# PowerfulGhost/gguf-triton-kernel

Measured on AMD Instinct MI355X. Metric: effective fp16 TFLOPS (+ quant-weight GB/s) per GGUF type, higher is better.
Workload: dtype f16; 1 GPU; q8_0_4096x4096_m128; gguf_type=q8_0, N_out=4096, K=4096, parallelism=single, weight_copies=61, weight_bytes_rotated=1087373312, graphs_rotated=1

## Files before the change

### gguf-triton-kernel_amd/csrc/gguf_internal.hpp

```cpp
#pragma once
#include <hip/hip_runtime.h>
#include <stdint.h>

namespace gq {

struct Tuning {
    long long blas_min_tokens = 768;
    long long gemm_max_bytes = 1LL << 31;
    int gemm_i8 = 0;
    int fused_decode = 1;
    int decode_f8_itc = 1;
    int decode_q6_img = -1;
    int gemm_aq = 1;
    int gemm_rg = 0;
    long long gemm_splits = 0;
    int gemm_partial_f32 = 0;
    int skinny = -1;
    int skinny_rg = 0;
    int rgemm = -1;
    int sgemm = -1;
    int sgemm_splits = 0;
    int sgemm_streamk = -1;
    int rgemm_ilc = 0;
    int sgemm_full = -1;
    int kstream = -1;
    int cus = 0;
    int ablate = 0;
};
const Tuning &tuning();
int set_tuning(const char *key, long long value);
void reset_tuning();
int num_cus();

enum ActMode : int { ACT_AOS = 0, ACT_SOA = 1, ACT_DEQ = 2, ACT_I8 = 3, ACT_F8 = 4, ACT_F8DEQ = 5 };
enum ActForm : int { AF_F16 = 0, AF_I8 = 1 };

hipError_t launch_quant_blocks(int kind, const void *x, void *y, int64_t nblocks, hipStream_t s);

hipError_t launch_act_quant(int mode, const uint16_t *X, int64_t ldx, int64_t rows, int64_t K, void *out0,
                            void *out1, void *out2, hipStream_t s);
constexpr int kMaxDeqSegs = 8;
struct DeqSeg {
    const uint16_t *X;
    int64_t ldx, rows, K;
    uint16_t *xdeq;
    int64_t wg0;
};
hipError_t launch_act_quant_deq_grouped(const DeqSeg *segs, int n, hipStream_t s, int mode = ACT_DEQ);

hipError_t launch_gemv(int fmt, const uint8_t *A, const int8_t *xq, const float *xd, const float *xs, uint16_t *C,
                       int64_t M, int64_t N, int64_t K, int64_t ldc, hipStream_t s);

bool decode_fused_ok(int fmt, int64_t N, int64_t K, bool fp8 = false);
hipError_t launch_decode_fused(int fmt, const uint8_t *A, const uint16_t *X, int64_t ldx, uint16_t *C, int64_t M,
                               int64_t N, int64_t K, int64_t ldc, hipStream_t s, bool fp8 = false);

struct GemmPlan {
    int nb = 8;
    int rg = 2;
    int splits = 1;
    int chunks_per_split = 1;
    int act = AF_F16;
    int loaders = 0;
    int pf16 = 0;
    int aq = 0;
    size_t partial_bytes = 0;
};
struct GemmAct {
    const uint16_t *xdeq = nullptr;
    const int8_t *xq = nullptr;
    const float *xd = nullptr;
    int64_t ldd = 0;
    const uint16_t *xraw = nullptr;
    int64_t ldx = 0;
};
bool gemm_aq_ok(const GemmPlan &p);
bool gemm_supported(int fmt, int64_t K);
GemmPlan plan_gemm(int fmt, int64_t M, int64_t N, int64_t K, int act = AF_F16);
hipError_t launch_gemm(int fmt, const uint8_t *A, const GemmAct &x, uint16_t *C, float *partials,
                       const GemmPlan &plan, int64_t M, int64_t N, int64_t K, int64_t ldc, hipStream_t s);

hipError_t launch_gemm_reduce_f16(int nb, int rg, const uint16_t *P, uint16_t *C, int64_t M, int64_t N, int64_t ldc,
                                  int S, int tiles_x, int tiles_y, hipStream_t s);

struct RGemmPlan {
    bool ok = false;
    int nb = 8, tiles_m = 0, tiles_n = 0, splits = 1;
    size_t partial_bytes = 0;
};

RGemmPlan plan_rgemm(int64_t M, int64_t N, int64_t K);
bool rgemm_ilc(int fmt, const RGemmPlan &p);
unsigned int ilc_timeouts();
unsigned int kstream_timeouts();
int rgemm_per_cu(int fmt, int nb);
hipError_t launch_rgemm(int fmt, int aq, const uint8_t *A, const uint16_t *X, int64_t ldx, uint16_t *C, void *partials,
                        const RGemmPlan &p, int64_t M, int64_t N, int64_t K, int64_t ldc, hipStream_t s);
RGemmPlan plan_sgemm(int64_t M, int64_t N, int64_t K, int splits);
bool sgemm_ilc(const RGemmPlan &p);
hipError_t launch_sgemm(int fmt, const uint8_t *A, const uint16_t *X, uint16_t *C, void *partials, const RGemmPlan &p,
                        int64_t M, int64_t N, int64_t K, int64_t ldc, hipStream_t s);

struct SGroupItem {
    int fmt;
    const uint8_t *A;
    const uint16_t *X;
    uint16_t *C;
    int64_t ldc, M, K;
};
struct SGroupPlan {
    bool ok = false;
    int nb = 8, tiles_n = 1, blocks = 0;
    int tiles_m[16] = {}, splits[16] = {}, wg0[16] = {};
    bool streamk = false;
    int U = 0;
    int ustart[16] = {}, scap[16] = {};
    int cost[16] = {}, cstart[16] = {};
    size_t poff[16] = {};
    size_t foff[16] = {}, noff[16] = {};
    size_t partial_bytes = 0;
};
SGroupPlan plan_sgemm_grouped(const SGroupItem *items, int n, int64_t N, int splits);
hipError_t launch_sgemm_grouped(const SGroupItem *items, int n, int64_t N, const SGroupPlan &g, void *partials,
                                hipStream_t s);

struct DecodeItem {
    int fmt;
    const uint8_t *A;
    const uint16_t *X;
    int64_t ldx;
    uint16_t *C;
    int64_t ldc;
    int64_t M, K;
};
bool decode_grouped_ok(const DecodeItem *items, int n, int64_t N, bool fp8 = false);
hipError_t launch_decode_grouped(const DecodeItem *items, int n, int64_t N, hipStream_t s, bool fp8 = false);

constexpr int kMaxIdPairs = 64;
bool decode_id_ok(int fmt, int64_t M, int64_t pairs, int64_t K);
hipError_t launch_decode_id(int fmt, const uint8_t *A, const int32_t *ids, const uint16_t *B, uint16_t *C, int64_t E,
                            int64_t M, int64_t N, int64_t S, int64_t K, int64_t ldb, int64_t ldb_slot, int64_t ldc,
                            hipStream_t s);

bool decode_id_glu_ok(int fmt, int64_t M, int64_t pairs, int64_t K);
hipError_t launch_decode_id_glu(int fmt, const uint8_t *A_gate, const uint8_t *A_up, const int32_t *ids, const uint16_t *B,
// ... 60 lines not shown
```

### gguf-triton-kernel_amd/csrc/gq_capi.hip

```cpp
#include <climits>
#include <cstdio>
#include <dlfcn.h>
#include <mutex>
#include <cstdarg>
#include <cstdlib>
#include <string>

#include <rccl/rccl.h>

#include "../../include/gguf_mmq.h"
#include "gguf_blocks.hpp"
#include "gguf_internal.hpp"

namespace gq {
namespace {

Tuning g_tuning;
std::once_flag g_tuning_once;

bool parse_key(Tuning &t, const char *key, long long v)
{
    auto in = [&](std::initializer_list<long long> ok) {
        for (long long o : ok)
            if (v == o) return true;
        return false;
    };
    const std::string k = key;
    if (k == "GQ_BLAS_MIN_TOKENS") t.blas_min_tokens = v;
    else if (k == "GQ_GEMM_MAX_BYTES") {
        if (v <= 0) return false;
        t.gemm_max_bytes = v < (1LL << 31) ? v : (1LL << 31);
    } else if (k == "GQ_GEMM_I8") t.gemm_i8 = v != 0;
    else if (k == "GQ_NO_FUSED_DECODE") t.fused_decode = v == 0;
    else if (k == "GQ_DECODE_F8_ITC") t.decode_f8_itc = v != 0;
    else if (k == "GQ_SGEMM_STREAMK") t.sgemm_streamk = v < 0 ? -1 : (v != 0);
    else if (k == "GQ_DECODE_Q6_IMG") {
        if (!in({-1, 0, 1})) return false;
        t.decode_q6_img = (int)v;
    }
    else if (k == "GQ_GEMM_AQ") t.gemm_aq = v != 0;
    else if (k == "GQ_GEMM_RG") {
        if (!in({0, 1, 2})) return false;
        t.gemm_rg = (int)v;
    } else if (k == "GQ_GEMM_SPLITS") {
        if (v < 0) return false;
        t.gemm_splits = v;
    } else if (k == "GQ_GEMM_PARTIAL") t.gemm_partial_f32 = v != 0;
    else if (k == "GQ_SKINNY") {
        if (!in({-1, 0, 1})) return false;
        t.skinny = (int)v;
    } else if (k == "GQ_SKINNY_RG") {
        if (!in({0, 1, 2, 3, 4})) return false;
        t.skinny_rg = (int)v;
    } else if (k == "GQ_RGEMM") {
        if (!in({-1, 0, 1})) return false;
        t.rgemm = (int)v;
    } else if (k == "GQ_SGEMM") {
        if (!in({-1, 0, 1})) return false;
        t.sgemm = (int)v;
    } else if (k == "GQ_SGEMM_SPLITS") {
        if (v < 0 || v > 4096) return false;
        t.sgemm_splits = (int)v;
    } else if (k == "GQ_RGEMM_ILC") t.rgemm_ilc = v != 0;
    else if (k == "GQ_SGEMM_FULL") {
        t.sgemm_full = v < 0 ? -1 : (v != 0);
    } else if (k == "GQ_CUS") {
        if (v < 0 || v > 1024) return false;
        t.cus = (int)v;
    } else if (k == "GQ_KSTREAM") {
        if (!in({-1, 0, 1})) return false;
        t.kstream = (int)v;
    } else if (k == "GQ_ABLATE") t.ablate = (int)v;
    else return false;
    return true;
}

void tuning_from_env(Tuning &t)
{
    t = Tuning{};
    static const char *const keys[] = {"GQ_BLAS_MIN_TOKENS", "GQ_GEMM_MAX_BYTES", "GQ_GEMM_I8", "GQ_NO_FUSED_DECODE",
                                       "GQ_DECODE_Q6_IMG", "GQ_DECODE_F8_ITC", "GQ_GEMM_AQ", "GQ_GEMM_RG", "GQ_GEMM_SPLITS",
                                       "GQ_GEMM_PARTIAL", "GQ_SKINNY", "GQ_SKINNY_RG", "GQ_RGEMM", "GQ_SGEMM",
                                       "GQ_SGEMM_SPLITS", "GQ_SGEMM_STREAMK", "GQ_RGEMM_ILC", "GQ_SGEMM_FULL", "GQ_CUS",
                                       "GQ_KSTREAM", "GQ_ABLATE"};
    for (const char *k : keys) {
        const char *e = getenv(k);
        if (!e || !*e) continue;
        long long v;
        if (std::string(k) == "GQ_GEMM_PARTIAL") v = std::string(e) == "f32";
        else v = atoll(e);
        if (!parse_key(t, k, v)) fprintf(stderr, "gguf_mmq: ignoring %s=%s (out of range)\n", k, e);
    }
}

}

const Tuning &tuning()
{
    std::call_once(g_tuning_once, [] { tuning_from_env(g_tuning); });
    return g_tuning;
}

int set_tuning(const char *key, long long value)
{
    tuning();
    Tuning t = g_tuning;
    if (!key || !parse_key(t, key, value)) return -1;
    g_tuning = t;
    return 0;
}

void reset_tuning()
{
    tuning();
    Tuning t;
    tuning_from_env(t);
    g_tuning = t;
}

int num_cus()
{
    if (tuning().cus > 0) return tuning().cus;
    static int cached[64] = {0};
    int dev = 0;
    if (hipGetDevice(&dev) != hipSuccess || dev < 0 || dev >= 64) dev = 0;
    if (cached[dev] <= 0) {
        int n = 0;
        if (hipDeviceGetAttribute(&n, hipDeviceAttributeMultiprocessorCount, dev) != hipSuccess || n <= 0) n = 256;
        cached[dev] = n;
    }
    return cached[dev];
}

namespace {

struct TypeInfo {
// ... 1114 lines not shown
```

### gguf-triton-kernel_amd/csrc/mmq_rgemm.hip

```cpp
#include <algorithm>
#include <type_traits>

#include "gguf_blocks.hpp"
#include "gguf_internal.hpp"
#include "gguf_mfma.hpp"
#include "gguf_q8_1.hpp"

namespace gq {

#ifdef GQ_RGEMM_STAMPS
__device__ unsigned long long g_rstamps[65536][14];
#define GQ_RST(i) (st[i] = __builtin_amdgcn_s_memtime())
#else
#define GQ_RST(i) ((void)0)
#endif

__device__ unsigned int g_ilc_timeouts;

namespace {

#ifndef GQ_RGEMM_ABL
#define GQ_RGEMM_ABL 0
#endif
constexpr int ABL = GQ_RGEMM_ABL;

constexpr int RW = 8;
constexpr int RPRIO_WAVE = RW / 2;
constexpr int RRG = 2;
constexpr int RBM = 16 * RW * RRG;
constexpr int LDS_CAP = 160 * 1024;
constexpr int kSpol = 16;

template <int F> struct HImg;
template <> struct HImg<Q8_0> { static constexpr int NPH = 9; };
template <> struct HImg<Q4_K> { static constexpr int NPH = 5; };
template <> struct HImg<Q5_K> { static constexpr int NPH = 7; };
template <> struct HImg<Q3_K> { static constexpr int NPH = 5; };
template <> struct HImg<Q2_K> { static constexpr int NPH = 5; };
template <> struct HImg<Q4_0> { static constexpr int NPH = 5; };
#ifndef GQ_Q6_NPH
#define GQ_Q6_NPH 8
#endif
template <> struct HImg<Q6_K> { static constexpr int NPH = GQ_Q6_NPH; };
template <int F> __device__ __forceinline__ int hpos_swz(int r)
{
    return F == Q6_K && HImg<F>::NPH == 8 ? (r & 7) : 0;
}
template <int F> __device__ __forceinline__ uint32_t hsrc(int h, int pc)
{
    if constexpr (F == Q8_0) return 128u * h + 16u * pc;
    if constexpr (F == Q4_K) return pc == 0 ? 0u : 16u + 64u * h + 16u * (pc - 1);
    if constexpr (F == Q5_K) return pc < 3 ? 16u * pc : 48u + 64u * h + 16u * (pc - 3);
    if constexpr (F == Q3_K) return pc < 2 ? 16u * pc : (pc < 4 ? 32u + 32u * h + 16u * (pc - 2) : 94u);
    if constexpr (F == Q2_K) return pc == 0 || pc == 4 ? 0u : (pc < 3 ? 16u + 32u * h + 16u * (pc - 1) : 68u);
    if constexpr (F == Q4_0) return 64u * h + 16u * pc;
    return pc < 4 ? 64u * h + 16u * pc : (pc < 6 ? 128u + 32u * h + 16u * (pc - 4) : (pc == 6 ? 192u : 194u));
}

template <int F, int NB> struct RCfg {
    static constexpr int BN = 16 * NB;
    static constexpr int NPH = HImg<F>::NPH, HRB = 16 * NPH, SB = Layout<F>::BYTES * (256 / Layout<F>::QK);
    static constexpr int WW = 2 * 32 * HRB, WWI = WW / 1024, H0I = (32 * NPH + 63) / 64;
    static constexpr int X_OFF = RW * WW;
    static constexpr int X_BYTES = BN * 512;
    static constexpr int X_INSTR = X_BYTES / 1024;
    static constexpr int NX = X_INSTR / RW;
    static constexpr int LDS = X_OFF + X_BYTES;
    static_assert(WW % 1024 == 0 && X_INSTR % RW == 0, "whole DMA instructions per wave");
    static_assert(LDS <= LDS_CAP, "LDS budget");
};

template <int F> __device__ __forceinline__ int sub_elem(int u, int q)
{
    if constexpr (F == Q6_K) return 128 * (u >> 1) + 32 * (u & 1) + 64 * (q >> 2) + 8 * (q & 3);
    return 64 * u + 8 * q;
}

template <int F> __device__ __forceinline__ void block_piece(int kb, int j, int &u, int &q)
{
    if constexpr (F == Q6_K) {
        const int b4 = kb & 3;
        u = 2 * (kb >> 2) + (b4 & 1);
        q = 4 * (b4 >> 1) + j;
    } else {
// ... 150 lines not shown
                }
            }
#pragma unroll
            for (int g = 0; g < G; ++g) {
                if (s0 + g >= S) v[g] = (u32x4){0u, 0u, 0u, 0u};
#pragma unroll
                for (int j = 0; j < TPU; ++j) {
                    const uint32_t x0 = j == 0 ? v[g].x : v[g].z, x1 = j == 0 ? v[g].y : v[g].w;
                    acc[j][0] += h2f(x0 & 0xffffu) * up[g];
                    acc[j][1] += h2f(x0 >> 16) * up[g];
                    acc[j][2] += h2f(x1 & 0xffffu) * up[g];
                    acc[j][3] += h2f(x1 >> 16) * up[g];
                }
            }
        }
        const int64_t row = m0 + 16 * wr + 4 * (ln >> 4);
        if (row >= M) continue;
#pragma unroll
        for (int j = 0; j < TPU; ++j) {
            const int64_t tok = n0 + 16 * (TPU * u + j) + (ln & 15);
            if (tok >= N) continue;
            uint16_t *dst = C + tok * ldc + row;
            if (row + 4 <= M) {
                *(u32x2 *)dst = (u32x2){(uint32_t)f2h_bits(acc[j][0]) | ((uint32_t)f2h_bits(acc[j][1]) << 16),
                                        (uint32_t)f2h_bits(acc[j][2]) | ((uint32_t)f2h_bits(acc[j][3]) << 16)};
            } else {
                for (int e = 0; e < 4 && row + e < M; ++e) dst[e] = f2h_bits(acc[j][e]);
            }
        }
    }
}

template <int NB>
__device__ __forceinline__ void ilc_combine(uint16_t *__restrict__ C, uint16_t *__restrict__ P, int64_t M, int64_t N,
                                            int64_t ldc, const TileId &id, uint32_t nonce)
{
    constexpr int BN = 16 * NB;
    const int lane = threadIdx.x & 63, wave = __builtin_amdgcn_readfirstlane(threadIdx.x >> 6);
    const int gz = id.gz, z = id.z;
    const int64_t tile = (int64_t)id.y * id.gx + id.x;
    const IlcSync sy = ilc_sync(P, id, BN);
    asm volatile("s_waitcnt vmcnt(0)" ::: "memory");
    __syncthreads();
    if (wave == 0) {
        uint64_t *tf = sy.flags + tile * gz;
        if (lane == 0) __hip_atomic_store(tf + z, ilc_flag(nonce, gz, z), __ATOMIC_RELAXED, __HIP_MEMORY_SCOPE_AGENT);
        ilc_wait(tf, nonce, gz);
        if (lane == 0 && z == 0) __hip_atomic_store(sy.nonce + tile, nonce + 1u, __ATOMIC_RELAXED, __HIP_MEMORY_SCOPE_AGENT);
    }
    __syncthreads();
    ilc_sum<NB>(C, P, M, N, ldc, (int64_t)id.x * RBM, (int64_t)id.y * BN, tile, gz, (int64_t)id.gx * id.gy * gz, gz, z,
                gz);
}
template <int NB>
__device__ __forceinline__ void store_tile(const f32x4 (&acc)[RRG][NB], uint16_t *__restrict__ C,
                                           uint16_t *__restrict__ P, int64_t M, int64_t N, int64_t ldc, int spol,
                                           const TileId &id)
{
    constexpr int BN = 16 * NB;
    const int lane = threadIdx.x & 63, wave = __builtin_amdgcn_readfirstlane(threadIdx.x >> 6);
    const int g = lane >> 4, l16 = lane & 15;
    const int64_t m0 = (int64_t)id.x * RBM, n0 = (int64_t)id.y * BN;
    if (id.gz > 1) {
        const int64_t tile = (int64_t)id.y * id.gx + id.x;
        const int64_t bidx = tile * id.gz + id.z;
        float mx = 0.f;
#pragma unroll
        for (int rg = 0; rg < RRG; ++rg)
#pragma unroll
            for (int t = 0; t < NB; ++t)
#pragma unroll
                for (int i = 0; i < 4; ++i) mx = fmaxf(mx, fabsf(acc[rg][t][i]));
        int m = __builtin_bit_cast(int, mx);
        m = __builtin_bit_cast(int, fmaxf(__builtin_bit_cast(float, m), __builtin_bit_cast(float, __builtin_amdgcn_update_dpp(0, m, 0x111, 0xf, 0xf, true))));
        m = __builtin_bit_cast(int, fmaxf(__builtin_bit_cast(float, m), __builtin_bit_cast(float, __builtin_amdgcn_update_dpp(0, m, 0x112, 0xf, 0xf, true))));
        m = __builtin_bit_cast(int, fmaxf(__builtin_bit_cast(float, m), __builtin_bit_cast(float, __builtin_amdgcn_update_dpp(0, m, 0x114, 0xf, 0xf, true))));
        m = __builtin_bit_cast(int, fmaxf(__builtin_bit_cast(float, m), __builtin_bit_cast(float, __builtin_amdgcn_update_dpp(0, m, 0x118, 0xf, 0xf, true))));
        m = __builtin_bit_cast(int, fmaxf(__builtin_bit_cast(float, m), __builtin_bit_cast(float, __builtin_amdgcn_update_dpp(0, m, 0x142, 0xa, 0xf, true))));
        m = __builtin_bit_cast(int, fmaxf(__builtin_bit_cast(float, m), __builtin_bit_cast(float, __builtin_amdgcn_update_dpp(0, m, 0x143, 0xc, 0xf, true))));
        const uint32_t mb = (uint32_t)__builtin_amdgcn_readlane(m, 63);
        const int E = (int)((mb >> 23) & 0xff) - 127;
        const int e = E - 14 > 0 ? (E - 14 < 127 ? E - 14 : 126) : 0;
        const float down = __builtin_bit_cast(float, (uint32_t)(127 - e) << 23);
        const int64_t nblk = (int64_t)id.gx * id.gy * id.gz;
        const __amdgpu_buffer_rsrc_t prs = __builtin_amdgcn_make_buffer_rsrc(
            (void *)P, 0, (int)(uint32_t)(nblk * (RBM * BN * 2 + RW * 4)), 0x00020000);
        const uint32_t bo = (uint32_t)(bidx * (RBM * BN * 2));
        if (lane == 0) {
            const uint32_t eo = (uint32_t)(nblk * (RBM * BN * 2) + (bidx * RW + wave) * 4);
            if (spol == 2) __builtin_amdgcn_raw_buffer_store_b32((uint32_t)e, prs, eo, 0, 2);
            else if (spol == 16) __builtin_amdgcn_raw_buffer_store_b32((uint32_t)e, prs, eo, 0, 16);
            else __builtin_amdgcn_raw_buffer_store_b32((uint32_t)e, prs, eo, 0, 0);
        }
        auto pk = [down](const f32x4 &v) {
            return (u32x2){(uint32_t)f2h_bits(v[0] * down) | ((uint32_t)f2h_bits(v[1] * down) << 16),
                           (uint32_t)f2h_bits(v[2] * down) | ((uint32_t)f2h_bits(v[3] * down) << 16)};
        };
#pragma unroll
        for (int rg = 0; rg < RRG; ++rg) {
            if constexpr (NB == 1) {
                const uint32_t vo = bo + 8u * (uint32_t)((RRG * wave + rg) * 64 + lane);
                if (spol == 2) __builtin_amdgcn_raw_buffer_store_b64(pk(acc[rg][0]), prs, vo, 0, 2);
                else if (spol == 16) __builtin_amdgcn_raw_buffer_store_b64(pk(acc[rg][0]), prs, vo, 0, 16);
                else __builtin_amdgcn_raw_buffer_store_b64(pk(acc[rg][0]), prs, vo, 0, 0);
            } else {
#pragma unroll
                for (int uu = 0; uu < NB / 2; ++uu) {
                    const u32x2 lo = pk(acc[rg][2 * uu]), hi = pk(acc[rg][2 * uu + 1]);
                    const u32x4 w = {lo.x, lo.y, hi.x, hi.y};
                    const uint32_t vo = bo + 16u * (uint32_t)(((RRG * wave + rg) * (NB / 2) + uu) * 64 + lane);
                    if (spol == 2) __builtin_amdgcn_raw_buffer_store_b128(w, prs, vo, 0, 2);
                    else if (spol == 16) __builtin_amdgcn_raw_buffer_store_b128(w, prs, vo, 0, 16);
                    else __builtin_amdgcn_raw_buffer_store_b128(w, prs, vo, 0, 0);
                }
            }
        }
        return;
    }
#pragma unroll
    for (int rg = 0; rg < RRG; ++rg) {
        const int64_t row = m0 + 16 * (RRG * wave + rg) + 4 * g;
        if (row >= M) continue;
#pragma unroll
        for (int t = 0; t < NB; ++t) {
            const int64_t tok = n0 + 16 * t + l16;
            if (tok >= N) continue;
            const f32x4 v = acc[rg][t];
            uint16_t *dst = C + tok * ldc + row;
            if (row + 4 <= M) {
                *(u32x2 *)dst = (u32x2){(uint32_t)f2h_bits(v[0]) | ((uint32_t)f2h_bits(v[1]) << 16),
                                        (uint32_t)f2h_bits(v[2]) | ((uint32_t)f2h_bits(v[3]) << 16)};
            } else {
                for (int i = 0; i < 4 && row + i < M; ++i) dst[i] = f2h_bits(v[i]);
            }
        }
    }
}

template <int NB>
__device__ __forceinline__ void store_tile_rows(const f32x4 (&acc)[RRG][NB], uint16_t *__restrict__ C,
                                                const int32_t *__restrict__ rowmap, int64_t M, int64_t N, int64_t ldc,
                                                const TileId &id)
{
    const int lane = threadIdx.x & 63, wave = __builtin_amdgcn_readfirstlane(threadIdx.x >> 6);
    const int g = lane >> 4, l16 = lane & 15;
    const int64_t m0 = (int64_t)id.x * RBM;
#pragma unroll
    for (int t = 0; t < NB; ++t) {
        const int tok = 16 * t + l16;
        if (tok >= N) continue;
        uint16_t *out = C + (int64_t)rowmap[tok] * ldc;
#pragma unroll
        for (int rg = 0; rg < RRG; ++rg) {
            const int64_t row = m0 + 16 * (RRG * wave + rg) + 4 * g;
            if (row >= M) continue;
            const f32x4 v = acc[rg][t];
            uint16_t *dst = out + row;
            if (row + 4 <= M) {
                *(u32x2 *)dst = (u32x2){(uint32_t)f2h_bits(v[0]) | ((uint32_t)f2h_bits(v[1]) << 16),
                                        (uint32_t)f2h_bits(v[2]) | ((uint32_t)f2h_bits(v[3]) << 16)};
            } else {
                for (int i = 0; i < 4 && row + i < M; ++i) dst[i] = f2h_bits(v[i]);
            }
        }
    }
}

template <int F, int NB, int AQ>
__global__ __launch_bounds__(64 * RW) void rgemm_kernel(const uint8_t *__restrict__ A, const uint16_t *__restrict__ X,
                                                       int64_t ldx, uint16_t *__restrict__ C, uint16_t *__restrict__ P,
                                                       int64_t M, int64_t N, int64_t K, int64_t ldc, int spol,
                                                       int ilc_gx, int ilc_gy)
{
    using G = RCfg<F, NB>;
    __shared__ __attribute__((aligned(1024))) uint8_t lds[G::LDS];
    const int tid = threadIdx.x, lane = tid & 63;
    const int wave = __builtin_amdgcn_readfirstlane(tid >> 6);
    const bool ilc = ilc_gx > 0;
    if (wave >= RPRIO_WAVE) __builtin_amdgcn_s_setprio(1);
    const TileId tile = ilc ? ilc_tile(ilc_gx, ilc_gy) : grid_tile();
    const int64_t m0 = (int64_t)tile.x * RBM, n0 = (int64_t)tile.y * G::BN, sb = tile.z;
    const int64_t row_bytes = (K / Layout<F>::QK) * Layout<F>::BYTES;
    uint8_t *const ximg = lds + G::X_OFF;
#ifdef GQ_RGEMM_STAMPS
    unsigned long long st[14] = {};
    st[0] = __builtin_amdgcn_s_memrealtime();
    GQ_RST(1);
#endif
    const uint32_t nonce = ilc_nonce(P, tile, G::BN, ilc);

    u32x4 xv[AQ ? NB : 1];
    if constexpr (AQ != 0 && !(ABL & 2)) {
        const __amdgpu_buffer_rsrc_t xrs =
            __builtin_amdgcn_make_buffer_rsrc((void *)X, 0, (int)(uint32_t)(((N - 1) * ldx + K) * 2), 0x00020000);
#pragma unroll
        for (int ps = 0; ps < NB; ++ps) {
            const int b = 128 * ps + (tid >> 2), r = b >> 3, kb = b & 7;
            const int64_t tok = n0 + r < N ? n0 + r : N - 1;
            xv[ps] = __builtin_amdgcn_raw_buffer_load_b128(
                xrs, (uint32_t)(tok * ldx * 2) + 2u * (uint32_t)(256 * sb + 32 * kb + 8 * (lane & 3)), 0, 0);
        }
    }

    const __amdgpu_buffer_rsrc_t wrs =
        __builtin_amdgcn_make_buffer_rsrc((void *)A, 0, (int)(uint32_t)((M * row_bytes + 15) & ~(int64_t)15), 0x00020000);
    uint8_t *const wimg = lds + wave * G::WW;
    auto issue_w = [&](auto i0c, auto i1c) __attribute__((always_inline)) {
        constexpr int I0 = decltype(i0c)::value, I1 = decltype(i1c)::value;
        if constexpr (ABL & 1) return;
#pragma unroll
        for (int i = I0; i < I1; ++i) {
            const int p = 64 * i + lane, h = p / (32 * G::NPH), rem = p - h * (32 * G::NPH);
            const int r = rem / G::NPH, pc = (rem - r * G::NPH) ^ hpos_swz<F>(r);
            const int64_t row = m0 + 32 * wave + r < M ? m0 + 32 * wave + r : M - 1;
            dma16(wrs, wimg + 1024 * i, (uint32_t)(row * row_bytes) + hsrc<F>(h, pc), (uint32_t)(G::SB * sb));
        }
    };
    auto issue_x = [&]() __attribute__((always_inline)) {
        if constexpr (AQ != 0 || (ABL & 2)) return;
        const __amdgpu_buffer_rsrc_t xrs =
            __builtin_amdgcn_make_buffer_rsrc((void *)X, 0, (int)(uint32_t)(N * K * 2), 0x00020000);
#pragma unroll
        for (int i = 0; i < G::NX; ++i) {
            const int k = wave + RW * i, pp = 64 * k + lane;
            const int u = pp / (G::BN * 8), r = (pp / 8) % G::BN, qd = pp & 7, q = qd ^ act_swz(r);
            const int64_t tok = n0 + r < N ? n0 + r : N - 1;
            const uint32_t vo = (uint32_t)(tok * K * 2) + 2u * (uint32_t)sub_elem<F>(u, q);
            dma16(xrs, lds + G::X_OFF + 1024 * k, vo, (uint32_t)(512 * sb));
        }
    };
#ifndef GQ_RGEMM_WPRE
#define GQ_RGEMM_WPRE 2
#endif
    constexpr int WPRE = AQ != 0 && GQ_RGEMM_WPRE < G::WWI ? GQ_RGEMM_WPRE : G::WWI;
    issue_x();
    issue_w(std::integral_constant<int, 0>{}, std::integral_constant<int, WPRE>{});
    GQ_RST(2);

    if constexpr (AQ != 0 && !(ABL & 2)) {
#pragma unroll
        for (int ps = 0; ps < NB; ++ps) {
            const int b = 128 * ps + (tid >> 2), r = b >> 3, kb = b & 7;
            u32x4 o;
            if constexpr (AQ == 2) {
                const F8Quad fq = f8_quad(xv[ps]);
                o = (u32x4){fq.xt[0], fq.xt[1], fq.xt[2], fq.xt[3]};
            } else {
                o = deq_quad(xv[ps]);
            }
            int u, q;
            block_piece<F>(kb, lane & 3, u, q);
            *(u32x4 *)(ximg + u * (G::BN * 128) + 128 * r + 16 * (q ^ act_swz(r))) = o;
        }
    }
    issue_w(std::integral_constant<int, WPRE>{}, std::integral_constant<int, G::WWI>{});
    constexpr int WN = (ABL & 1) ? 0 : G::WWI;
    asm volatile("s_waitcnt vmcnt(%0) lgkmcnt(0)" ::"n"(WN) : "memory");
    GQ_RST(3);
    __builtin_amdgcn_s_barrier();
    GQ_RST(4);

    f32x4 acc[RRG][NB];
#pragma unroll
    for (int rg = 0; rg < RRG; ++rg)
#pragma unroll
        for (int t = 0; t < NB; ++t) acc[rg][t] = (f32x4){0.f, 0.f, 0.f, 0.f};
    constexpr int H1N = (ABL & 1) ? 0 : G::WWI - G::H0I;
    asm volatile("s_waitcnt vmcnt(%0)" ::"n"(H1N) : "memory");
    GQ_RST(5);
#pragma unroll
    for (int u = 0; u < 4 && !(ABL & 4); ++u) {
        if (u == 2) {
#ifdef GQ_RGEMM_STAMPS
            asm volatile("s_waitcnt lgkmcnt(0)" ::: "memory");
            for (int rg = 0; rg < RRG; ++rg)
                for (int t = 0; t < NB; ++t) asm volatile("" ::"v"(acc[rg][t]));
#endif
            GQ_RST(6);
            asm volatile("s_waitcnt vmcnt(0)" ::: "memory");
            GQ_RST(7);
        }
        mul_substage<F, NB>(wimg + (u >> 1) * (32 * G::HRB), ximg + u * (G::BN * 128), u, acc, 0);
    }
#ifdef GQ_RGEMM_STAMPS
    for (int rg = 0; rg < RRG; ++rg)
        for (int t = 0; t < NB; ++t) asm volatile("" ::"v"(acc[rg][t]));
#endif
    GQ_RST(8);
    if constexpr ((ABL & 4) != 0) asm volatile("s_waitcnt vmcnt(0)" ::: "memory");

    if constexpr ((ABL & 8) != 0) {
        if (acc[0][0][0] == 1234.5f) C[0] = 0;
        return;
    }
    store_tile<NB>(acc, C, P, M, N, ldc, ilc ? 16 : spol, tile);
    if (ilc && tile.gz > 1) ilc_combine<NB>(C, P, M, N, ldc, tile, nonce);
#ifdef GQ_RGEMM_STAMPS
    GQ_RST(9);
    asm volatile("s_waitcnt vmcnt(0)" ::: "memory");
    GQ_RST(10);
    st[11] = __builtin_amdgcn_s_memrealtime();
    const int wg = (int)(blockIdx.x + gridDim.x * (blockIdx.y + gridDim.y * blockIdx.z));
    st[12] = (unsigned long long)wg;
    unsigned xcc;
    asm volatile("s_getreg_b32 %0, hwreg(HW_REG_XCC_ID)" : "=s"(xcc));
    st[13] = xcc & 0xfu;
    const int id = wg * RW + wave;
    if (lane == 0 && id < 65536)
        for (int i = 0; i < 14; ++i) g_rstamps[id][i] = st[i];
#endif
}

#ifndef GQ_SGEMM_NSMAX
#define GQ_SGEMM_NSMAX 6
#endif
constexpr int SG_NSMAX = GQ_SGEMM_NSMAX;
template <int F, int NB> struct SCfg {
    static constexpr int BN = 16 * NB;
    static constexpr int NPH = HImg<F>::NPH, HRB = 16 * NPH, SB = Layout<F>::BYTES * (256 / Layout<F>::QK);
    static constexpr int W_BYTES = RBM * HRB, X_BYTES = BN * 256;
    static constexpr int SLOT = W_BYTES + X_BYTES;
    static constexpr int WH_INSTR = (RBM * NPH + 63) / 64, NWH = (WH_INSTR + RW - 1) / RW;
    static constexpr int XH_INSTR = X_BYTES / 1024, NXH = (XH_INSTR + RW - 1) / RW;
    static constexpr int NPS = ((ABL & 1) ? 0 : NWH) + ((ABL & 2) ? 0 : NXH);
    static constexpr bool PAD = WH_INSTR % RW != 0 || XH_INSTR % RW != 0 || XH_INSTR < RW;
    static constexpr int NS = (LDS_CAP - 1024) / SLOT > SG_NSMAX ? SG_NSMAX : (LDS_CAP - 1024) / SLOT;
    static constexpr int SCRATCH = NS * SLOT;
    static constexpr int LDS = SCRATCH + (PAD ? 1024 : 0);
    static_assert(NS >= 2, "two ring slots");
    static_assert(LDS <= LDS_CAP, "LDS budget");
    static_assert((NS - 2) * NPS <= 63, "vmcnt range");
};

constexpr int kMaxSParts = 16;
struct SPart {
    int fmt;
    const uint8_t *A;
    const uint16_t *X;
    uint16_t *C, *P;
    int64_t M, K, ldc;
    int tiles_m, tiles_n, splits, wg0;
    int ustart, scap;
    int cost, cstart;
    uint64_t *flags;
    uint32_t *nonce;
};
struct SParts {
    int n;
// ... 433 lines not shown
                acc[j][0] += h2f(x0 & 0xffffu) * up[k];
                acc[j][1] += h2f(x0 >> 16) * up[k];
                acc[j][2] += h2f(x1 & 0xffffu) * up[k];
                acc[j][3] += h2f(x1 >> 16) * up[k];
            }
        }
    }
    const int64_t row = m0 + 16 * wr + 4 * (lane >> 4);
    if (row >= q.M) return;
#pragma unroll
    for (int j = 0; j < TPU; ++j) {
        const int64_t tok = n0 + 16 * (TPU * u + j) + (lane & 15);
        if (tok >= a.N) continue;
        uint16_t *dst = q.C + tok * q.ldc + row;
        if (row + 4 <= q.M) {
            *(u32x2 *)dst = (u32x2){(uint32_t)f2h_bits(acc[j][0]) | ((uint32_t)f2h_bits(acc[j][1]) << 16),
                                    (uint32_t)f2h_bits(acc[j][2]) | ((uint32_t)f2h_bits(acc[j][3]) << 16)};
        } else {
            for (int e = 0; e < 4 && row + e < q.M; ++e) dst[e] = f2h_bits(acc[j][e]);
        }
    }
}

template <int F, int NB>
hipError_t launch_snb(const uint8_t *A, const uint16_t *X, uint16_t *C, void *P, const RGemmPlan &p, int64_t M,
                      int64_t N, int64_t K, int64_t ldc, hipStream_t s)
{
    static const int occ = [] {
        int n = 0;
        return hipOccupancyMaxActiveBlocksPerMultiprocessor(&n, sgemm_kernel<F, NB>, 64 * RW, 0) == hipSuccess ? n : 0;
    }();
    const int64_t blocks = (int64_t)p.tiles_m * p.tiles_n * p.splits;
    if (sgemm_ilc(p) && blocks <= (int64_t)num_cus() * occ) {
        sgemm_kernel<F, NB><<<dim3((unsigned)blocks), dim3(64 * RW), 0, s>>>(A, X, C, (uint16_t *)P, M, N, K, ldc, 16,
                                                                             tuning().sgemm_full != 0, p.tiles_m, p.tiles_n, 1);
        return hipGetLastError();
    }
#ifndef GQ_SGEMM_ZORDER
#define GQ_SGEMM_ZORDER 1
#endif
    if (GQ_SGEMM_ZORDER && p.splits > 1 && (blocks & 7) == 0 && N * K * 2 > ((int64_t)4 << 20)) {
        sgemm_kernel<F, NB><<<dim3((unsigned)blocks), dim3(64 * RW), 0, s>>>(A, X, C, (uint16_t *)P, M, N, K, ldc, kSpol,
                                                                             tuning().sgemm_full != 0, p.tiles_m, p.tiles_n, 2);
    } else {
        const dim3 grid((unsigned)p.tiles_m, (unsigned)p.tiles_n, (unsigned)p.splits);
        sgemm_kernel<F, NB><<<grid, dim3(64 * RW), 0, s>>>(A, X, C, (uint16_t *)P, M, N, K, ldc, kSpol,
                                                            tuning().sgemm_full != 0, 0, 0, 0);
    }
    hipError_t e = hipGetLastError();
    if (e != hipSuccess || p.splits == 1) return e;
    return launch_gemm_reduce_f16(NB, RRG, (const uint16_t *)P, C, M, N, ldc, p.splits, p.tiles_m, p.tiles_n, s);
}

template <int F, int NB, int AQ>
hipError_t launch_nb(const uint8_t *A, const uint16_t *X, int64_t ldx, uint16_t *C, void *P, const RGemmPlan &p,
                     int64_t M, int64_t N, int64_t K, int64_t ldc, hipStream_t s)
{
    static const int occ = [] {
        int n = 0;
        return hipOccupancyMaxActiveBlocksPerMultiprocessor(&n, rgemm_kernel<F, NB, AQ>, 64 * RW, 0) == hipSuccess ? n : 0;
    }();
    const int64_t blocks = (int64_t)p.tiles_m * p.tiles_n * p.splits;
    if (rgemm_ilc(F, p) && blocks <= (int64_t)num_cus() * occ) {
        rgemm_kernel<F, NB, AQ><<<dim3((unsigned)blocks), dim3(64 * RW), 0, s>>>(A, X, ldx, C, (uint16_t *)P, M, N, K, ldc,
                                                                                 16, p.tiles_m, p.tiles_n);
        return hipGetLastError();
    }
    const dim3 grid((unsigned)p.tiles_m, (unsigned)p.tiles_n, (unsigned)p.splits);
    rgemm_kernel<F, NB, AQ><<<grid, dim3(64 * RW), 0, s>>>(A, X, ldx, C, (uint16_t *)P, M, N, K, ldc, kSpol,
                                                           0, 0);
    hipError_t e = hipGetLastError();
    if (e != hipSuccess || p.splits == 1) return e;
    return launch_gemm_reduce_f16(NB, RRG, (const uint16_t *)P, C, M, N, ldc, p.splits, p.tiles_m, p.tiles_n, s);
}

template <int F, int AQ>
hipError_t launch_f(const uint8_t *A, const uint16_t *X, int64_t ldx, uint16_t *C, void *P, const RGemmPlan &p,
                    int64_t M, int64_t N, int64_t K, int64_t ldc, hipStream_t s)
{
    switch (p.nb) {
    case 1: return launch_nb<F, 1, AQ>(A, X, ldx, C, P, p, M, N, K, ldc, s);
    case 2: return launch_nb<F, 2, AQ>(A, X, ldx, C, P, p, M, N, K, ldc, s);
    case 4: return launch_nb<F, 4, AQ>(A, X, ldx, C, P, p, M, N, K, ldc, s);
    case 8: return launch_nb<F, 8, AQ>(A, X, ldx, C, P, p, M, N, K, ldc, s);
    default: return hipErrorInvalidValue;
    }
}

}

int rgemm_per_cu(int fmt, int nb)
{
#define GQ_RPC(F)                                                                                                      \
    switch (nb) {                                                                                                      \
    case 1: return LDS_CAP / RCfg<F, 1>::LDS;                                                                          \
    case 2: return LDS_CAP / RCfg<F, 2>::LDS;                                                                          \
    case 4: return LDS_CAP / RCfg<F, 4>::LDS;                                                                          \
    default: return LDS_CAP / RCfg<F, 8>::LDS;                                                                         \
    }
    switch (fmt) {
    case Q8_0: GQ_RPC(Q8_0)
    case Q4_K: GQ_RPC(Q4_K)
    case Q6_K: GQ_RPC(Q6_K)
    default: return 0;
    }
#undef GQ_RPC
}

RGemmPlan plan_rgemm(int64_t M, int64_t N, int64_t K)
{
    RGemmPlan p;
    if (M < 1 || N < 1 || K < 256 || K % 256 != 0) return p;
    p.nb = N > 64 ? 8 : (N > 32 ? 4 : (N > 16 ? 2 : 1));
    p.tiles_m = (int)((M + RBM - 1) / RBM);
    p.tiles_n = (int)((N + 16 * p.nb - 1) / (16 * p.nb));
    p.splits = (int)(K / 256);
    const int64_t tiles = (int64_t)p.tiles_m * p.tiles_n, nblk = tiles * p.splits;
    p.partial_bytes = p.splits > 1 ? ilc_flags_off(nblk, 16 * p.nb) + ilc_sync_bytes(nblk, tiles) : 0;
    p.ok = true;
    return p;
}

bool rgemm_ilc(int fmt, const RGemmPlan &p)
{
    if (!p.ok || p.splits < 2 || tuning().rgemm_ilc == 0) return false;
    return (int64_t)p.tiles_m * p.tiles_n * p.splits <= (int64_t)num_cus() * rgemm_per_cu(fmt, p.nb);
}

bool sgemm_ilc(const RGemmPlan &p)
{
    if (!p.ok || p.splits < 2 || tuning().rgemm_ilc == 0) return false;
    return (int64_t)p.tiles_m * p.tiles_n * p.splits <= (int64_t)num_cus();
}

unsigned int ilc_timeouts()
{
    unsigned int v = 0;
    return hipMemcpyFromSymbol(&v, HIP_SYMBOL(g_ilc_timeouts), sizeof(v)) == hipSuccess ? v : ~0u;
}

RGemmPlan plan_sgemm(int64_t M, int64_t N, int64_t K, int splits)
{
    RGemmPlan p;
    if (M < 1 || N < 1 || K < 256 || K % 256 != 0) return p;
    p.nb = N > 64 ? 8 : (N > 32 ? 4 : (N > 16 ? 2 : 1));
    p.tiles_m = (int)((M + RBM - 1) / RBM);
    p.tiles_n = (int)((N + 16 * p.nb - 1) / (16 * p.nb));
    const int64_t tiles = (int64_t)p.tiles_m * p.tiles_n, nsb = K / 256, cus = num_cus();
    int64_t S = splits > 0 ? splits : (tiles >= cus ? 1 : cus / tiles);
    if (S > nsb) S = nsb;
    p.splits = (int)(S < 1 ? 1 : S);
    const int64_t nblk = tiles * p.splits;
    p.partial_bytes = p.splits > 1 ? ilc_flags_off(nblk, 16 * p.nb) + ilc_sync_bytes(nblk, tiles) : 0;
    p.ok = true;
    return p;
}

hipError_t launch_sgemm(int fmt, const uint8_t *A, const uint16_t *X, uint16_t *C, void *partials, const RGemmPlan &p,
                        int64_t M, int64_t N, int64_t K, int64_t ldc, hipStream_t s)
{
    if (!p.ok) return hipErrorInvalidValue;
    return dispatch_fmt(fmt, [&](auto f) {
        constexpr int F = decltype(f)::value;
        switch (p.nb) {
        case 1: return launch_snb<F, 1>(A, X, C, partials, p, M, N, K, ldc, s);
        case 2: return launch_snb<F, 2>(A, X, C, partials, p, M, N, K, ldc, s);
        case 4: return launch_snb<F, 4>(A, X, C, partials, p, M, N, K, ldc, s);
        case 8: return launch_snb<F, 8>(A, X, C, partials, p, M, N, K, ldc, s);
        default: return hipErrorInvalidValue;
        }
    });
}

SortedPlan plan_sgemm_id(int64_t E, int64_t M, int64_t P, int64_t K)
{
    SortedPlan p;
    if (E < 1 || E > kMaxSortExperts || M < 1 || P < 1 || P > kMaxSortPairs || K < 256 || K % 256 != 0) return p;
    const int64_t ne = E < P ? E : P, avg = (P + ne - 1) / ne;
    p.nb = avg > 64 ? 8 : (avg > 32 ? 4 : (avg > 16 ? 2 : 1));
// ... 212 lines not shown
```

Baseline: 274.1 TFLOP/s.

## Overlap rgemm epilogue stores with the second-half MFMAs per token group

```diff
diff --git a/gguf-triton-kernel_amd/csrc/gguf_internal.hpp b/gguf-triton-kernel_amd/csrc/gguf_internal.hpp
--- a/gguf-triton-kernel_amd/csrc/gguf_internal.hpp
+++ b/gguf-triton-kernel_amd/csrc/gguf_internal.hpp
@@ -22,6 +22,7 @@
     int sgemm_splits = 0;
     int sgemm_streamk = -1;
     int rgemm_ilc = 0;
+    int rgemm_estore = -1;
     int sgemm_full = -1;
     int kstream = -1;
     int cus = 0;
@@ -91,6 +92,7 @@
 
 RGemmPlan plan_rgemm(int64_t M, int64_t N, int64_t K);
 bool rgemm_ilc(int fmt, const RGemmPlan &p);
+bool rgemm_estore(int nb);
 unsigned int ilc_timeouts();
 unsigned int kstream_timeouts();
 int rgemm_per_cu(int fmt, int nb);
diff --git a/gguf-triton-kernel_amd/csrc/gq_capi.hip b/gguf-triton-kernel_amd/csrc/gq_capi.hip
--- a/gguf-triton-kernel_amd/csrc/gq_capi.hip
+++ b/gguf-triton-kernel_amd/csrc/gq_capi.hip
@@ -62,7 +62,10 @@
         if (v < 0 || v > 4096) return false;
         t.sgemm_splits = (int)v;
     } else if (k == "GQ_RGEMM_ILC") t.rgemm_ilc = v != 0;
-    else if (k == "GQ_SGEMM_FULL") {
+    else if (k == "GQ_RGEMM_ESTORE") {
+        if (!in({-1, 0, 1})) return false;
+        t.rgemm_estore = (int)v;
+    } else if (k == "GQ_SGEMM_FULL") {
         t.sgemm_full = v < 0 ? -1 : (v != 0);
     } else if (k == "GQ_CUS") {
         if (v < 0 || v > 1024) return false;
@@ -81,7 +84,7 @@
     static const char *const keys[] = {"GQ_BLAS_MIN_TOKENS", "GQ_GEMM_MAX_BYTES", "GQ_GEMM_I8", "GQ_NO_FUSED_DECODE",
                                        "GQ_DECODE_Q6_IMG", "GQ_DECODE_F8_ITC", "GQ_GEMM_AQ", "GQ_GEMM_RG", "GQ_GEMM_SPLITS",
                                        "GQ_GEMM_PARTIAL", "GQ_SKINNY", "GQ_SKINNY_RG", "GQ_RGEMM", "GQ_SGEMM",
-                                       "GQ_SGEMM_SPLITS", "GQ_SGEMM_STREAMK", "GQ_RGEMM_ILC", "GQ_SGEMM_FULL", "GQ_CUS",
+                                       "GQ_SGEMM_SPLITS", "GQ_SGEMM_STREAMK", "GQ_RGEMM_ILC", "GQ_RGEMM_ESTORE", "GQ_SGEMM_FULL", "GQ_CUS",
                                        "GQ_KSTREAM", "GQ_ABLATE"};
     for (const char *k : keys) {
         const char *e = getenv(k);
diff --git a/gguf-triton-kernel_amd/csrc/mmq_rgemm.hip b/gguf-triton-kernel_amd/csrc/mmq_rgemm.hip
--- a/gguf-triton-kernel_amd/csrc/mmq_rgemm.hip
+++ b/gguf-triton-kernel_amd/csrc/mmq_rgemm.hip
@@ -11,8 +11,10 @@
 #ifdef GQ_RGEMM_STAMPS
 __device__ unsigned long long g_rstamps[65536][14];
 #define GQ_RST(i) (st[i] = __builtin_amdgcn_s_memtime())
+#define GQ_RST_PTR(i) (&st[i])
 #else
 #define GQ_RST(i) ((void)0)
+#define GQ_RST_PTR(i) nullptr
 #endif
 
 __device__ unsigned int g_ilc_timeouts;
@@ -30,6 +32,7 @@
 constexpr int RBM = 16 * RW * RRG;
 constexpr int LDS_CAP = 160 * 1024;
 constexpr int kSpol = 16;
+constexpr int kEstoreAutoNb = 2;
 
 template <int F> struct HImg;
 template <> struct HImg<Q8_0> { static constexpr int NPH = 9; };
@@ -286,46 +289,53 @@
     ilc_sum<NB>(C, P, M, N, ldc, (int64_t)id.x * RBM, (int64_t)id.y * BN, tile, gz, (int64_t)id.gx * id.gy * gz, gz, z,
                 gz);
 }
-template <int NB>
-__device__ __forceinline__ void store_tile(const f32x4 (&acc)[RRG][NB], uint16_t *__restrict__ C,
-                                           uint16_t *__restrict__ P, int64_t M, int64_t N, int64_t ldc, int spol,
-                                           const TileId &id)
-{
-    constexpr int BN = 16 * NB;
-    const int lane = threadIdx.x & 63, wave = __builtin_amdgcn_readfirstlane(threadIdx.x >> 6);
-    const int g = lane >> 4, l16 = lane & 15;
-    const int64_t m0 = (int64_t)id.x * RBM, n0 = (int64_t)id.y * BN;
-    if (id.gz > 1) {
-        const int64_t tile = (int64_t)id.y * id.gx + id.x;
-        const int64_t bidx = tile * id.gz + id.z;
-        float mx = 0.f;
-#pragma unroll
-        for (int rg = 0; rg < RRG; ++rg)
-#pragma unroll
-            for (int t = 0; t < NB; ++t)
-#pragma unroll
-                for (int i = 0; i < 4; ++i) mx = fmaxf(mx, fabsf(acc[rg][t][i]));
-        int m = __builtin_bit_cast(int, mx);
-        m = __builtin_bit_cast(int, fmaxf(__builtin_bit_cast(float, m), __builtin_bit_cast(float, __builtin_amdgcn_update_dpp(0, m, 0x111, 0xf, 0xf, true))));
-        m = __builtin_bit_cast(int, fmaxf(__builtin_bit_cast(float, m), __builtin_bit_cast(float, __builtin_amdgcn_update_dpp(0, m, 0x112, 0xf, 0xf, true))));
-        m = __builtin_bit_cast(int, fmaxf(__builtin_bit_cast(float, m), __builtin_bit_cast(float, __builtin_amdgcn_update_dpp(0, m, 0x114, 0xf, 0xf, true))));
-        m = __builtin_bit_cast(int, fmaxf(__builtin_bit_cast(float, m), __builtin_bit_cast(float, __builtin_amdgcn_update_dpp(0, m, 0x118, 0xf, 0xf, true))));
-        m = __builtin_bit_cast(int, fmaxf(__builtin_bit_cast(float, m), __builtin_bit_cast(float, __builtin_amdgcn_update_dpp(0, m, 0x142, 0xa, 0xf, true))));
-        m = __builtin_bit_cast(int, fmaxf(__builtin_bit_cast(float, m), __builtin_bit_cast(float, __builtin_amdgcn_update_dpp(0, m, 0x143, 0xc, 0xf, true))));
-        const uint32_t mb = (uint32_t)__builtin_amdgcn_readlane(m, 63);
-        const int E = (int)((mb >> 23) & 0xff) - 127;
-        const int e = E - 14 > 0 ? (E - 14 < 127 ? E - 14 : 126) : 0;
-        const float down = __builtin_bit_cast(float, (uint32_t)(127 - e) << 23);
+__device__ __forceinline__ int wave_exponent(float mx)
+{
+    int m = __builtin_bit_cast(int, mx);
+    m = __builtin_bit_cast(int, fmaxf(__builtin_bit_cast(float, m), __builtin_bit_cast(float, __builtin_amdgcn_update_dpp(0, m, 0x111, 0xf, 0xf, true))));
+    m = __builtin_bit_cast(int, fmaxf(__builtin_bit_cast(float, m), __builtin_bit_cast(float, __builtin_amdgcn_update_dpp(0, m, 0x112, 0xf, 0xf, true))));
+    m = __builtin_bit_cast(int, fmaxf(__builtin_bit_cast(float, m), __builtin_bit_cast(float, __builtin_amdgcn_update_dpp(0, m, 0x114, 0xf, 0xf, true))));
+    m = __builtin_bit_cast(int, fmaxf(__builtin_bit_cast(float, m), __builtin_bit_cast(float, __builtin_amdgcn_update_dpp(0, m, 0x118, 0xf, 0xf, true))));
+    m = __builtin_bit_cast(int, fmaxf(__builtin_bit_cast(float, m), __builtin_bit_cast(float, __builtin_amdgcn_update_dpp(0, m, 0x142, 0xa, 0xf, true))));
+    m = __builtin_bit_cast(int, fmaxf(__builtin_bit_cast(float, m), __builtin_bit_cast(float, __builtin_amdgcn_update_dpp(0, m, 0x143, 0xc, 0xf, true))));
+    const uint32_t mb = (uint32_t)__builtin_amdgcn_readlane(m, 63);
+    const int E = (int)((mb >> 23) & 0xff) - 127;
+    return E - 14 > 0 ? (E - 14 < 127 ? E - 14 : 126) : 0;
+}
+template <int NB> __device__ __forceinline__ float tile_absmax(const f32x4 (&acc)[RRG][NB], int t0, int t1, float mx)
+{
+#pragma unroll
+    for (int rg = 0; rg < RRG; ++rg)
+#pragma unroll
+        for (int t = t0; t < t1; ++t)
+#pragma unroll
+            for (int i = 0; i < 4; ++i) mx = fmaxf(mx, fabsf(acc[rg][t][i]));
+    return mx;
+}
+template <int NB, int SP = -1> struct PartBlock {
+    __amdgpu_buffer_rsrc_t prs;
+    uint32_t bo, eo;
+    int spol;
+    __device__ __forceinline__ PartBlock(uint16_t *P, const TileId &id, int spol_) : spol(SP < 0 ? spol_ : SP)
+    {
+        constexpr int BN = 16 * NB;
+        const int wave = __builtin_amdgcn_readfirstlane(threadIdx.x >> 6);
+        const int64_t bidx = ((int64_t)id.y * id.gx + id.x) * id.gz + id.z;
         const int64_t nblk = (int64_t)id.gx * id.gy * id.gz;
-        const __amdgpu_buffer_rsrc_t prs = __builtin_amdgcn_make_buffer_rsrc(
-            (void *)P, 0, (int)(uint32_t)(nblk * (RBM * BN * 2 + RW * 4)), 0x00020000);
-        const uint32_t bo = (uint32_t)(bidx * (RBM * BN * 2));
-        if (lane == 0) {
-            const uint32_t eo = (uint32_t)(nblk * (RBM * BN * 2) + (bidx * RW + wave) * 4);
-            if (spol == 2) __builtin_amdgcn_raw_buffer_store_b32((uint32_t)e, prs, eo, 0, 2);
-            else if (spol == 16) __builtin_amdgcn_raw_buffer_store_b32((uint32_t)e, prs, eo, 0, 16);
-            else __builtin_amdgcn_raw_buffer_store_b32((uint32_t)e, prs, eo, 0, 0);
-        }
+        prs = __builtin_amdgcn_make_buffer_rsrc((void *)P, 0, (int)(uint32_t)(nblk * (RBM * BN * 2 + RW * 4)), 0x00020000);
+        bo = (uint32_t)(bidx * (RBM * BN * 2));
+        eo = (uint32_t)(nblk * (RBM * BN * 2) + (bidx * RW + wave) * 4);
+    }
+    __device__ __forceinline__ void exponent(int e) const
+    {
+        if ((threadIdx.x & 63) != 0) return;
+        if (spol == 2) __builtin_amdgcn_raw_buffer_store_b32((uint32_t)e, prs, eo, 0, 2);
+        else if (spol == 16) __builtin_amdgcn_raw_buffer_store_b32((uint32_t)e, prs, eo, 0, 16);
+        else __builtin_amdgcn_raw_buffer_store_b32((uint32_t)e, prs, eo, 0, 0);
+    }
+    __device__ __forceinline__ void tiles(const f32x4 (&acc)[RRG][NB], int t0, int t1, float down) const
+    {
+        const int lane = threadIdx.x & 63, wave = __builtin_amdgcn_readfirstlane(threadIdx.x >> 6);
         auto pk = [down](const f32x4 &v) {
             return (u32x2){(uint32_t)f2h_bits(v[0] * down) | ((uint32_t)f2h_bits(v[1] * down) << 16),
                            (uint32_t)f2h_bits(v[2] * down) | ((uint32_t)f2h_bits(v[3] * down) << 16)};
@@ -339,7 +349,7 @@
                 else __builtin_amdgcn_raw_buffer_store_b64(pk(acc[rg][0]), prs, vo, 0, 0);
             } else {
 #pragma unroll
-                for (int uu = 0; uu < NB / 2; ++uu) {
+                for (int uu = t0 / 2; uu < t1 / 2; ++uu) {
                     const u32x2 lo = pk(acc[rg][2 * uu]), hi = pk(acc[rg][2 * uu + 1]);
                     const u32x4 w = {lo.x, lo.y, hi.x, hi.y};
                     const uint32_t vo = bo + 16u * (uint32_t)(((RRG * wave + rg) * (NB / 2) + uu) * 64 + lane);
@@ -349,14 +359,21 @@
                 }
             }
         }
-        return;
-    }
+    }
+};
+template <int NB>
+__device__ __forceinline__ void store_c_tiles(const f32x4 (&acc)[RRG][NB], int t0, int t1, uint16_t *__restrict__ C,
+                                              int64_t M, int64_t N, int64_t ldc, const TileId &id)
+{
+    const int lane = threadIdx.x & 63, wave = __builtin_amdgcn_readfirstlane(threadIdx.x >> 6);
+    const int g = lane >> 4, l16 = lane & 15;
+    const int64_t m0 = (int64_t)id.x * RBM, n0 = (int64_t)id.y * (16 * NB);
 #pragma unroll
     for (int rg = 0; rg < RRG; ++rg) {
         const int64_t row = m0 + 16 * (RRG * wave + rg) + 4 * g;
         if (row >= M) continue;
 #pragma unroll
-        for (int t = 0; t < NB; ++t) {
+        for (int t = t0; t < t1; ++t) {
             const int64_t tok = n0 + 16 * t + l16;
             if (tok >= N) continue;
             const f32x4 v = acc[rg][t];
@@ -369,6 +386,90 @@
             }
         }
     }
+}
+template <int NB>
+__device__ __forceinline__ void store_tile(const f32x4 (&acc)[RRG][NB], uint16_t *__restrict__ C,
+                                           uint16_t *__restrict__ P, int64_t M, int64_t N, int64_t ldc, int spol,
+                                           const TileId &id)
+{
+    if (id.gz > 1) {
+        const int e = wave_exponent(tile_absmax<NB>(acc, 0, NB, 0.f));
+        const PartBlock<NB> pb(P, id, spol);
+        pb.exponent(e);
+        pb.tiles(acc, 0, NB, __builtin_bit_cast(float, (uint32_t)(127 - e) << 23));
+        return;
+    }
+    store_c_tiles<NB>(acc, 0, NB, C, M, N, ldc, id);
+}
+
+#ifndef GQ_RGEMM_EGRP
+#define GQ_RGEMM_EGRP 2
+#endif
+template <int F, int NB, int SP>
+__device__ __forceinline__ void mul_half1_early(const uint8_t *wimg1, const uint8_t *xs2, f32x4 (&acc)[RRG][NB],
+                                                uint16_t *__restrict__ C, uint16_t *__restrict__ P, int64_t M,
+                                                int64_t N, int64_t ldc, const TileId &id,
+                                                unsigned long long *mfma_done)
+{
+    constexpr int BN = 16 * NB, GT = GQ_RGEMM_EGRP < NB ? GQ_RGEMM_EGRP : NB;
+    static_assert(GT % 2 == 0 && NB % GT == 0, "whole 16-byte units per group, whole groups per tile");
+    const int lane = threadIdx.x & 63;
+    const int g = lane >> 4, l16 = lane & 15;
+    f16x8 af[2][RRG][2];
+#pragma unroll
+    for (int v = 0; v < 2; ++v)
+#pragma unroll
+        for (int rg = 0; rg < RRG; ++rg)
+            half_frags<F>(wimg1 + (16 * HImg<F>::NPH) * (16 * rg + l16), g, 2 + v, l16, af[v][rg]);
+    const PartBlock<NB, SP> pb(P, id, SP);
+    float mx = 0.f;
+    auto groups = [&](auto split) __attribute__((always_inline)) {
+#pragma unroll
+        for (int t0 = 0; t0 < NB; t0 += GT) {
+#pragma unroll
+            for (int v = 0; v < 2; ++v) {
+#pragma unroll
+                for (int s = 0; s < 2; ++s) {
+                    f16x8 bk[GT];
+#pragma unroll
+                    for (int t = 0; t < GT; ++t) {
+                        const int r = 16 * (t0 + t) + l16;
+                        bk[t] = *(const f16x8 *)(xs2 + v * (BN * 128) + 128 * r + 16 * ((4 * s + g) ^ act_swz(r)));
+                    }
+#pragma unroll
+                    for (int rg = 0; rg < RRG; ++rg)
+#pragma unroll
+                        for (int t = 0; t < GT; ++t)
+                            acc[rg][t0 + t] =
+                                __builtin_amdgcn_mfma_f32_16x16x32_f16(af[v][rg][s], bk[t], acc[rg][t0 + t], 0, 0, 0);
+                }
+            }
+            if (mfma_done != nullptr && t0 + GT == NB) {
+#pragma unroll
+                for (int rg = 0; rg < RRG; ++rg)
+#pragma unroll
+                    for (int t = 0; t < GT; ++t) asm volatile("" ::"v"(acc[rg][t0 + t]));
+                *mfma_done = __builtin_amdgcn_s_memtime();
+            }
+            if constexpr (decltype(split)::value) {
+                mx = tile_absmax<NB>(acc, t0, t0 + GT, mx);
+                pb.tiles(acc, t0, t0 + GT, 1.f);
+            } else {
+                store_c_tiles<NB>(acc, t0, t0 + GT, C, M, N, ldc, id);
+            }
+        }
+    };
+    if (id.gz == 1) {
+        groups(std::false_type{});
+        return;
+    }
+    groups(std::true_type{});
+    const int e = wave_exponent(mx);
+    if (e != 0) {
+        asm volatile("s_waitcnt vmcnt(0)" ::: "memory");
+        pb.tiles(acc, 0, NB, __builtin_bit_cast(float, (uint32_t)(127 - e) << 23));
+    }
+    pb.exponent(e);
 }
 
 template <int NB>
@@ -400,7 +501,7 @@
     }
 }
 
-template <int F, int NB, int AQ>
+template <int F, int NB, int AQ, int ES = 0>
 __global__ __launch_bounds__(64 * RW) void rgemm_kernel(const uint8_t *__restrict__ A, const uint16_t *__restrict__ X,
                                                        int64_t ldx, uint16_t *__restrict__ C, uint16_t *__restrict__ P,
                                                        int64_t M, int64_t N, int64_t K, int64_t ldc, int spol,
@@ -502,32 +603,43 @@
     constexpr int H1N = (ABL & 1) ? 0 : G::WWI - G::H0I;
     asm volatile("s_waitcnt vmcnt(%0)" ::"n"(H1N) : "memory");
     GQ_RST(5);
-#pragma unroll
-    for (int u = 0; u < 4 && !(ABL & 4); ++u) {
-        if (u == 2) {
+    static_assert(ES == 0 || (NB > 1 && ABL == 0), "the early-store form: two token tiles or more, no ablation");
+    auto half1_landed = [&]() __attribute__((always_inline)) {
 #ifdef GQ_RGEMM_STAMPS
-            asm volatile("s_waitcnt lgkmcnt(0)" ::: "memory");
-            for (int rg = 0; rg < RRG; ++rg)
-                for (int t = 0; t < NB; ++t) asm volatile("" ::"v"(acc[rg][t]));
+        asm volatile("s_waitcnt lgkmcnt(0)" ::: "memory");
+        for (int rg = 0; rg < RRG; ++rg)
+            for (int t = 0; t < NB; ++t) asm volatile("" ::"v"(acc[rg][t]));
 #endif
-            GQ_RST(6);
-            asm volatile("s_waitcnt vmcnt(0)" ::: "memory");
-            GQ_RST(7);
-        }
-        mul_substage<F, NB>(wimg + (u >> 1) * (32 * G::HRB), ximg + u * (G::BN * 128), u, acc, 0);
-    }
+        GQ_RST(6);
+        asm volatile("s_waitcnt vmcnt(0)" ::: "memory");
+        GQ_RST(7);
+    };
+    if constexpr (ES != 0) {
+#pragma unroll
+        for (int u = 0; u < 2; ++u) mul_substage<F, NB>(wimg, ximg + u * (G::BN * 128), u, acc, 0);
+        half1_landed();
+        static_assert(kSpol == 16, "the early stores take one policy, at compile time: the launches' and the combine's");
+        mul_half1_early<F, NB, kSpol>(wimg + 32 * G::HRB, ximg + 2 * (G::BN * 128), acc, C, P, M, N, ldc, tile,
+                                      GQ_RST_PTR(8));
+    } else {
+#pragma unroll
+        for (int u = 0; u < 4 && !(ABL & 4); ++u) {
+            if (u == 2) half1_landed();
+            mul_substage<F, NB>(wimg + (u >> 1) * (32 * G::HRB), ximg + u * (G::BN * 128), u, acc, 0);
+        }
 #ifdef GQ_RGEMM_STAMPS
-    for (int rg = 0; rg < RRG; ++rg)
-        for (int t = 0; t < NB; ++t) asm volatile("" ::"v"(acc[rg][t]));
+        for (int rg = 0; rg < RRG; ++rg)
+            for (int t = 0; t < NB; ++t) asm volatile("" ::"v"(acc[rg][t]));
 #endif
-    GQ_RST(8);
-    if constexpr ((ABL & 4) != 0) asm volatile("s_waitcnt vmcnt(0)" ::: "memory");
-
-    if constexpr ((ABL & 8) != 0) {
-        if (acc[0][0][0] == 1234.5f) C[0] = 0;
-        return;
-    }
-    store_tile<NB>(acc, C, P, M, N, ldc, ilc ? 16 : spol, tile);
+        GQ_RST(8);
+        if constexpr ((ABL & 4) != 0) asm volatile("s_waitcnt vmcnt(0)" ::: "memory");
+
+        if constexpr ((ABL & 8) != 0) {
+            if (acc[0][0][0] == 1234.5f) C[0] = 0;
+            return;
+        }
+        store_tile<NB>(acc, C, P, M, N, ldc, ilc ? 16 : spol, tile);
+    }
     if (ilc && tile.gz > 1) ilc_combine<NB>(C, P, M, N, ldc, tile, nonce);
 #ifdef GQ_RGEMM_STAMPS
     GQ_RST(9);
@@ -1067,26 +1179,34 @@
     return launch_gemm_reduce_f16(NB, RRG, (const uint16_t *)P, C, M, N, ldc, p.splits, p.tiles_m, p.tiles_n, s);
 }
 
+template <int F, int NB, int AQ, int ES>
+hipError_t launch_es(const uint8_t *A, const uint16_t *X, int64_t ldx, uint16_t *C, void *P, const RGemmPlan &p,
+                     int64_t M, int64_t N, int64_t K, int64_t ldc, hipStream_t s)
+{
+    static const int occ = [] {
+        int n = 0;
+        return hipOccupancyMaxActiveBlocksPerMultiprocessor(&n, rgemm_kernel<F, NB, AQ, ES>, 64 * RW, 0) == hipSuccess ? n : 0;
+    }();
+    const int64_t blocks = (int64_t)p.tiles_m * p.tiles_n * p.splits;
+    if (rgemm_ilc(F, p) && blocks <= (int64_t)num_cus() * occ) {
+        rgemm_kernel<F, NB, AQ, ES><<<dim3((unsigned)blocks), dim3(64 * RW), 0, s>>>(A, X, ldx, C, (uint16_t *)P, M, N, K,
+                                                                                     ldc, 16, p.tiles_m, p.tiles_n);
+        return hipGetLastError();
+    }
+    const dim3 grid((unsigned)p.tiles_m, (unsigned)p.tiles_n, (unsigned)p.splits);
+    rgemm_kernel<F, NB, AQ, ES><<<grid, dim3(64 * RW), 0, s>>>(A, X, ldx, C, (uint16_t *)P, M, N, K, ldc, kSpol, 0, 0);
+    hipError_t e = hipGetLastError();
+    if (e != hipSuccess || p.splits == 1) return e;
+    return launch_gemm_reduce_f16(NB, RRG, (const uint16_t *)P, C, M, N, ldc, p.splits, p.tiles_m, p.tiles_n, s);
+}
+
 template <int F, int NB, int AQ>
 hipError_t launch_nb(const uint8_t *A, const uint16_t *X, int64_t ldx, uint16_t *C, void *P, const RGemmPlan &p,
                      int64_t M, int64_t N, int64_t K, int64_t ldc, hipStream_t s)
 {
-    static const int occ = [] {
-        int n = 0;
-        return hipOccupancyMaxActiveBlocksPerMultiprocessor(&n, rgemm_kernel<F, NB, AQ>, 64 * RW, 0) == hipSuccess ? n : 0;
-    }();
-    const int64_t blocks = (int64_t)p.tiles_m * p.tiles_n * p.splits;
-    if (rgemm_ilc(F, p) && blocks <= (int64_t)num_cus() * occ) {
-        rgemm_kernel<F, NB, AQ><<<dim3((unsigned)blocks), dim3(64 * RW), 0, s>>>(A, X, ldx, C, (uint16_t *)P, M, N, K, ldc,
-                                                                                 16, p.tiles_m, p.tiles_n);
-        return hipGetLastError();
-    }
-    const dim3 grid((unsigned)p.tiles_m, (unsigned)p.tiles_n, (unsigned)p.splits);
-    rgemm_kernel<F, NB, AQ><<<grid, dim3(64 * RW), 0, s>>>(A, X, ldx, C, (uint16_t *)P, M, N, K, ldc, kSpol,
-                                                           0, 0);
-    hipError_t e = hipGetLastError();
-    if (e != hipSuccess || p.splits == 1) return e;
-    return launch_gemm_reduce_f16(NB, RRG, (const uint16_t *)P, C, M, N, ldc, p.splits, p.tiles_m, p.tiles_n, s);
+    if constexpr (NB > 1 && ABL == 0)
+        if (rgemm_estore(NB)) return launch_es<F, NB, AQ, 1>(A, X, ldx, C, P, p, M, N, K, ldc, s);
+    return launch_es<F, NB, AQ, 0>(A, X, ldx, C, P, p, M, N, K, ldc, s);
 }
 
 template <int F, int AQ>
@@ -1140,6 +1260,12 @@
 {
     if (!p.ok || p.splits < 2 || tuning().rgemm_ilc == 0) return false;
     return (int64_t)p.tiles_m * p.tiles_n * p.splits <= (int64_t)num_cus() * rgemm_per_cu(fmt, p.nb);
+}
+
+bool rgemm_estore(int nb)
+{
+    const int v = tuning().rgemm_estore;
+    return nb > 1 && (v < 0 ? nb >= kEstoreAutoNb : v != 0);
 }
 
 bool sgemm_ilc(const RGemmPlan &p)
```

After: 291.1 TFLOP/s, median of 6. 6.2% higher.
